# gmum/3d-point-clouds-autocomplete

Measured on AMD Instinct MI355X. Metric: train-step point-clouds/sec at B=64, N=2048 (Chamfer+EMD), higher is better.
Workload: dtype f32 storage / accumulation / results; matrix products formed from f16 x2 (bf16 x3) pieces of the fp32 operands — NOT IEEE-fp32 products: the all-fp32-kernel step is `value_strict_fp32`

## Files before the change

3d-point-clouds-autocomplete_amd/csrc/conv_pp.hip:

```cpp
#include "hp_common.h"
#include "hp_conv_split.h"
#include <algorithm>
#include <cstdlib>
#include <type_traits>

namespace {

typedef _Float16 f16x8 __attribute__((ext_vector_type(8)));
typedef _Float16 f16x4 __attribute__((ext_vector_type(4)));
typedef _Float16 f16x2 __attribute__((ext_vector_type(2)));
typedef float f32x16 __attribute__((ext_vector_type(16)));
typedef float f32x4 __attribute__((ext_vector_type(4)));
typedef unsigned int u32x4 __attribute__((ext_vector_type(4)));
typedef unsigned int u32x2 __attribute__((ext_vector_type(2)));

constexpr int kTarget = 14;
constexpr int kExpMax = HP_PP_EXP_MAX;

__device__ __forceinline__ int frexp_exp(unsigned bits) {
    const int E = (int)((bits >> 23) & 0xff);
    return E ? E - 126 : 0;
}
__device__ __forceinline__ float pow2f(int e) {
    e = max(-126, min(127, e));
// ... 286 lines not shown
                            }
                        }
                    const float ov = __shfl_xor(best, 32, 64);
                    const int oi = __shfl_xor(bi, 32, 64);
                    if (ov > best || (ov == best && oi < bi)) {
                        best = ov;
                        bi = oi;
                    }
                    if (h == 0) {
                        cmax[(long)tile128 * p.N + col] = best;
                        cidx[(long)tile128 * p.N + col] = bi % p.group_rows;
                    }
                }
            }
            continue;
        }

        float m = 0.f;
        const float usA = pow2f(-ex), floor_v = p.relu ? 0.f : -__builtin_inff();
#pragma unroll
        for (int j = 0; j < TN; ++j)
#pragma unroll
            for (int e = 0; e < 16; e += 4) {
                const int cl = wn * 32 * TN + j * 32 + kmap(e, h);
                const f32x4 us4 = *reinterpret_cast<const f32x4*>(tab + cl), bv4 = *reinterpret_cast<const f32x4*>(tab + BN + cl);
#pragma unroll
                for (int u = 0; u < 4; ++u) {
                    const float us = us4[u] * usA;
#pragma unroll
                    for (int i = 0; i < 4; ++i) {
                        const float v = fmaxf(__builtin_fmaf(acc[i][j][e + u], us, bv4[u]), floor_v);
                        acc[i][j][e + u] = v;
                        m = fmaxf(m, fabsf(v));
                    }
                }
            }
#pragma unroll
        for (int o = 1; o < 64; o <<= 1) m = fmaxf(m, __shfl_xor(m, o, 64));
        if (lane == 0) xch[wid] = m;
        __syncthreads();
        m = fmaxf(fmaxf(xch[wm * 4], xch[wm * 4 + 1]), fmaxf(xch[wm * 4 + 2], xch[wm * 4 + 3]));
        const int eo = block_exp(m);
        if (wn == 0 && lane == 0 && row0 + wm * 128 < M) p.cexp[z * p.sWs + (long)tile128 * p.tiles_n + tile_n] = eo;
        const float sx = pow2f(eo);
        unsigned char* Cb = reinterpret_cast<unsigned char*>(p.C) + z * p.sWs * 4;
        const long crow = (long)p.N * 4;
#pragma unroll
        for (int i = 0; i < 4; ++i) {
            const int row = row0 + wm * 128 + i * 32 + r;
#pragma unroll
            for (int j = 0; j < TN; ++j) {
                unsigned H[4][2], L[4][2];
#pragma unroll
                for (int q = 0; q < 4; ++q)
#pragma unroll
                    for (int pr = 0; pr < 2; ++pr) {
                        const float x0 = acc[i][j][4 * q + 2 * pr] * sx, x1 = acc[i][j][4 * q + 2 * pr + 1] * sx;
                        H[q][pr] = pack2((_Float16)x0, (_Float16)x1);
                        L[q][pr] = lo_pair(x0, x1, H[q][pr]);
                    }
                unsigned char* line = Cb + (long)row * crow + (long)((col0 + wn * 32 * TN) / 32 + j) * 128 + (h << 4);
#pragma unroll
                for (int q = 0; q < 4; q += 2) {
#pragma unroll
                    for (int pr = 0; pr < 2; ++pr) {
                        auto s1 = __builtin_amdgcn_permlane32_swap(H[q][pr], H[q + 1][pr], false, false);
                        H[q][pr] = s1[0];
                        H[q + 1][pr] = s1[1];
                        auto s2 = __builtin_amdgcn_permlane32_swap(L[q][pr], L[q + 1][pr], false, false);
                        L[q][pr] = s2[0];
                        L[q + 1][pr] = s2[1];
                    }
                    if (row < M) {
                        *reinterpret_cast<u32x4*>(line + q * 16) = u32x4{H[q][0], H[q][1], H[q + 1][0], H[q + 1][1]};
                        *reinterpret_cast<u32x4*>(line + 64 + q * 16) = u32x4{L[q][0], L[q][1], L[q + 1][0], L[q + 1][1]};
                    }
                }
            }
        }
        __syncthreads();
    }
}

__global__ __launch_bounds__(256) void conv1_pp_kernel(const float* __restrict__ x, long sXz, const float* __restrict__ W, long sWz,
                                                       const float* __restrict__ b, long sBz, _Float16* __restrict__ h, int* __restrict__ hexp,
                                                       long sWs, long R) {
    __shared__ float smax[4];
    const int z = blockIdx.y;
    x += z * sXz; W += z * sWz; b += z * sBz;
    unsigned char* hb = reinterpret_cast<unsigned char*>(h) + z * sWs * 4;
    hexp += z * sWs;
    const int c4 = (threadIdx.x & 15) * 4;
    float w0[4], w1[4], w2[4], bb[4];
#pragma unroll
    for (int u = 0; u < 4; ++u) {
        w0[u] = W[(c4 + u) * 3];
        w1[u] = W[(c4 + u) * 3 + 1];
        w2[u] = W[(c4 + u) * 3 + 2];
        bb[u] = b[c4 + u];
    }
    for (long tile = blockIdx.x; tile * 128 < R; tile += gridDim.x) {
        const long base = tile * 128 + (threadIdx.x >> 4);
        float xv[8][3];
#pragma unroll
        for (int q = 0; q < 8; ++q) {
            const long row = min(base + 16 * q, R - 1);
            xv[q][0] = x[row * 3];
            xv[q][1] = x[row * 3 + 1];
            xv[q][2] = x[row * 3 + 2];
        }
        float o[8][4];
        float m = 0.f;
#pragma unroll
        for (int q = 0; q < 8; ++q)
#pragma unroll
            for (int u = 0; u < 4; ++u) {
                const float v = __builtin_fmaf(xv[q][2], w2[u], __builtin_fmaf(xv[q][1], w1[u], __builtin_fmaf(xv[q][0], w0[u], 0.f)));
                o[q][u] = fmaxf(v + bb[u], 0.f);
                if (base + 16 * q < R) m = fmaxf(m, o[q][u]);
            }
        m = hp::wave_max(m);
        __syncthreads();
        if ((threadIdx.x & 63) == 0) smax[threadIdx.x >> 6] = m;
        __syncthreads();
        const int eo = block_exp(fmaxf(fmaxf(smax[0], smax[1]), fmaxf(smax[2], smax[3])));
        if (threadIdx.x == 0) hexp[tile] = eo;
        const float sx = pow2f(eo);
#pragma unroll
        for (int q = 0; q < 8; ++q) {
            const long row = base + 16 * q;
            f16x4 hi, lo;
#pragma unroll
            for (int u = 0; u < 4; ++u) {
                const float xs = o[q][u] * sx;
                const _Float16 hh = (_Float16)xs;
                hi[u] = hh;
                lo[u] = (_Float16)(xs - (float)hh);
            }
            if (row < R) {
                unsigned char* line = hb + row * 256 + (c4 >> 5) * 128 + (c4 & 31) * 2;
                *reinterpret_cast<f16x4*>(line) = hi;
                *reinterpret_cast<f16x4*>(line + 64) = lo;
            }
        }
    }
}

__global__ __launch_bounds__(256) void pp_pack_kernel(const float* __restrict__ X, long M, int C, int cb, _Float16* __restrict__ P,
                                                      int* __restrict__ pexp) {
    __shared__ float smax[4];
    const int ncb = C / cb, blk = blockIdx.x % ncb;
    const long tile = blockIdx.x / ncb, r0 = tile * 128;
    const int rows = (int)min((long)128, M - r0);
    const int per_row = cb / 4;
    float m = 0.f;
    for (int i = threadIdx.x; i < rows * per_row; i += 256) {
        const int rr = i / per_row, c = blk * cb + (i % per_row) * 4;
        const f32x4 v = *reinterpret_cast<const f32x4*>(X + (r0 + rr) * C + c);
        m = fmaxf(fmaxf(m, fmaxf(fabsf(v[0]), fabsf(v[1]))), fmaxf(fabsf(v[2]), fabsf(v[3])));
    }
    m = hp::wave_max(m);
    if ((threadIdx.x & 63) == 0) smax[threadIdx.x >> 6] = m;
    __syncthreads();
    const int eo = block_exp(fmaxf(fmaxf(smax[0], smax[1]), fmaxf(smax[2], smax[3])));
    if (threadIdx.x == 0) pexp[tile * ncb + blk] = eo;
    const float sx = pow2f(eo);
    unsigned char* Pb = reinterpret_cast<unsigned char*>(P);
    for (int i = threadIdx.x; i < rows * per_row; i += 256) {
        const int rr = i / per_row, c = blk * cb + (i % per_row) * 4;
        const f32x4 v = *reinterpret_cast<const f32x4*>(X + (r0 + rr) * C + c);
        f16x4 hi, lo;
#pragma unroll
        for (int u = 0; u < 4; ++u) {
            const float xs = v[u] * sx;
            const _Float16 hh = (_Float16)xs;
            hi[u] = hh;
            lo[u] = (_Float16)(xs - (float)hh);
        }
        unsigned char* line = Pb + (r0 + rr) * (long)C * 4 + (c >> 5) * 128 + (c & 31) * 2;
        *reinterpret_cast<f16x4*>(line) = hi;
        *reinterpret_cast<f16x4*>(line + 64) = lo;
    }
}

__global__ __launch_bounds__(256) void pp_unpack_kernel(const _Float16* P, const int* __restrict__ pexp, long M, int C, int cb,
                                                        float* out, const int* __restrict__ fmt) {
    if (fmt && *fmt != HP_PP_FMT_P) return;
    const long nlines = M * (C / 32);
    const int ncb = C / cb;
    for (long ln = (long)blockIdx.x * 256 + threadIdx.x; ln < nlines; ln += (long)gridDim.x * 256) {
        const long row = ln / (C / 32);
        const int kt = (int)(ln % (C / 32));
        const u32x4* src = reinterpret_cast<const u32x4*>(reinterpret_cast<const unsigned char*>(P) + ln * 128);
        u32x4 w[8];
#pragma unroll
        for (int q = 0; q < 8; ++q) w[q] = src[q];
        const float us = pow2f(-pexp[(row >> 7) * ncb + (kt * 32) / cb]);
        f32x4* dst = reinterpret_cast<f32x4*>(reinterpret_cast<unsigned char*>(out) + ln * 128);
#pragma unroll
        for (int q = 0; q < 4; ++q) {
            const f16x8 hi = __builtin_bit_cast(f16x8, w[q]), lo = __builtin_bit_cast(f16x8, w[q + 4]);
            f32x4 a, b;
#pragma unroll
            for (int u = 0; u < 4; ++u) {
                a[u] = ((float)hi[u] + (float)lo[u]) * us;
                b[u] = ((float)hi[u + 4] + (float)lo[u + 4]) * us;
            }
            dst[2 * q] = a;
            dst[2 * q + 1] = b;
        }
    }
}

__global__ void pp_set_fmt_kernel(int* fmt, int v) { *fmt = v; }

hp::Switch g_presplit("HP_CONV_PRESPLIT", 1);

int pp_bn(int N) { return N >= 256 ? 256 : 128; }
int launch_pp(int mode, int n, const PpParams& p, hipStream_t stream) {
    const int bn = pp_bn(p.N);
    if (p.N % bn || p.K % 64 || p.M <= 0) return -1;
    PpParams q = p;
    q.tiles_n = p.N / bn;
    constexpr int kCus = 256;
    const bool small = mode == 0 && bn == 128;
    const int bm = small ? 128 : 256;
    const long tiles = (long)((p.M + bm - 1) / bm) * q.tiles_n;
    const int per_cu = small ? 2 : 1;
    long wgs = std::min<long>(tiles, kCus * per_cu / n > 0 ? kCus * per_cu / n : 1);
    const int mult = 8 * q.tiles_n / (q.tiles_n % 8 == 0 ? 8 : (8 % q.tiles_n == 0 ? q.tiles_n : 1));
    if (wgs >= mult) wgs = wgs / mult * mult;
    else wgs = (tiles >= q.tiles_n) ? q.tiles_n : wgs;
    const dim3 grid((unsigned)wgs, n);
    if (mode == 1) {
        if (bn == 256) hipLaunchKernelGGL((conv_pp_kernel<1, 2, 2>), grid, dim3(512), 0, stream, q);
        else hipLaunchKernelGGL((conv_pp_kernel<1, 1, 2>), grid, dim3(512), 0, stream, q);
    } else {
        if (bn == 256) hipLaunchKernelGGL((conv_pp_kernel<0, 2, 2>), grid, dim3(512), 0, stream, q);
        else hipLaunchKernelGGL((conv_pp_kernel<0, 1, 1>), grid, dim3(256), 0, stream, q);
    }
    HP_RETURN_LAST_ERROR();
}

}

bool hp_conv_presplit_enabled() { return g_presplit.get() != 0; }
int hp_conv_pp_ncb(int l) {
    static const int kC[5] = {0, 64, 128, 256, 512};
    return l <= 1 ? 1 : kC[l] / pp_bn(kC[l]);
}
HP_API int hp_conv_presplit_set(int on) { return g_presplit.set(on); }

static inline long pexp_off(int l, long tp) { return hp_conv_pp_exp_offset(l, tp); }

long hp_conv_pp_fmt_offset(long R) { return hp_conv_pp_exp_offset(5, hp_conv_split_tiles_pad(R)); }

int hp_conv_pp_layer1(int n, const float* x, long sXz, const float* W, long sWz, const float* b, long sBz, float* h1, float* area0,
                      long sWs, long R, hipStream_t stream) {
    const long tp = hp_conv_split_tiles_pad(R), blocks = (R + 127) / 128;
    hipLaunchKernelGGL(conv1_pp_kernel, dim3((unsigned)(blocks < 2048 ? blocks : 2048), n), dim3(256), 0, stream, x, sXz, W, sWz, b, sBz,
                       reinterpret_cast<_Float16*>(h1), reinterpret_cast<int*>(area0 + pexp_off(1, tp)), sWs, R);
    HP_RETURN_LAST_ERROR();
}

int hp_conv_pp_layer(int l, int n, const float* X, const float* bias, long sBiasz, float* C, float* area0, long sWs, long M,
                     float* cmax, int* cidx, int group_rows, hipStream_t stream) {
    static const int kRowsL[5] = {0, 128, 384, 896, 1408};
    static const long kWOffL[4] = {0, 8192, 40960, 172032};
    static const int kKL[4] = {64, 128, 256, 512};
    if (l < 2 || l > 5 || M <= 0) return -1;
    const long tp = hp_conv_split_tiles_pad(M);
    PpParams p{};
    p.A = reinterpret_cast<const _Float16*>(X);
    p.aexp = reinterpret_cast<const int*>(area0 + pexp_off(l - 1, tp));
    p.K = kKL[l - 2];
    p.a_ncb = hp_conv_pp_ncb(l - 1);
    p.a_kb_steps = p.K / 32 / p.a_ncb;
    p.Whl = reinterpret_cast<const _Float16*>(area0 + HP_CS_HI_OFF) + 2 * kWOffL[l - 2];
    p.wexp = reinterpret_cast<const int*>(area0 + HP_CS_WEXP_OFF) + kRowsL[l - 2];
    p.bias = bias; p.sBiasz = sBiasz;
    p.C = reinterpret_cast<_Float16*>(C);
    p.cexp = l < 5 ? reinterpret_cast<int*>(area0 + pexp_off(l, tp)) : nullptr;
    p.cmax = cmax; p.cidx = cidx;
    p.sWs = sWs;
    p.M = (int)M; p.N = kRowsL[l - 1] - kRowsL[l - 2];
    p.relu = l < 5; p.group_rows = group_rows;
    return launch_pp(l == 5 ? 1 : 0, n, p, stream);
}

int hp_conv_pp_mark(int n, float* area0, long sWs, long R, int fmt, hipStream_t stream) {
    for (int z = 0; z < n; ++z)
        hipLaunchKernelGGL(pp_set_fmt_kernel, dim3(1), dim3(1), 0, stream, reinterpret_cast<int*>(area0 + z * sWs + hp_conv_pp_fmt_offset(R)), fmt);
    HP_RETURN_LAST_ERROR();
}

int hp_conv_pp_unpack_ws(float* ws, long R, hipStream_t stream) {
    static const int kC[4] = {64, 128, 256, 512};
    const long tp = hp_conv_split_tiles_pad(R);
    float* area = ws + R * (64 + 128 + 256 + 512 + 512);
    int* fmt = reinterpret_cast<int*>(area + hp_conv_pp_fmt_offset(R));
    float* hl = ws;
    for (int l = 1; l <= 4; ++l) {
        const int C = kC[l - 1];
        const long lines = R * (C / 32);
        const unsigned blocks = (unsigned)std::min<long>((lines + 255) / 256, 8192);
        hipLaunchKernelGGL(pp_unpack_kernel, dim3(blocks), dim3(256), 0, stream, reinterpret_cast<const _Float16*>(hl),
                           reinterpret_cast<const int*>(area + pexp_off(l, tp)), R, C, C / hp_conv_pp_ncb(l), hl, fmt);
        hl += R * C;
    }
    hipLaunchKernelGGL(pp_set_fmt_kernel, dim3(1), dim3(1), 0, stream, fmt, HP_PP_FMT_F32);
    HP_RETURN_LAST_ERROR();
}

HP_API long hp_gemm_pp_workspace_floats(long M, int N, int K) {
    const long tiles = (M + 127) / 128;
    return M * K + tiles * 16 + N + (long)N * K + M * N + tiles * 16 + 2 * tiles * N + 64;
}
namespace {
struct PpWs {
    float *xp, *xexp, *wexp, *wp, *cp, *cexp, *cmax, *cidx;
};
PpWs pp_ws(float* ws, long M, int N, int K) {
    const long tiles = (M + 127) / 128;
    PpWs w;
    w.xp = ws;
    w.xexp = w.xp + M * K;
    w.wexp = w.xexp + tiles * 16;
    w.wp = w.wexp + N;
    w.cp = w.wp + (long)N * K;
    w.cexp = w.cp + M * N;
    w.cmax = w.cexp + tiles * 16;
    w.cidx = w.cmax + tiles * N;
    return w;
}
}
int hp_split_rows_launch(const float* W, int N, int K, float* hl, float* wexp, hipStream_t stream);

HP_API int hp_gemm_pp_prepare(long M, int N, int K, int xcb, const float* X, const float* W, float* ws, hipStream_t stream) {
    HP_CHECK_ARG(M > 0 && N > 0 && K > 0 && N % 128 == 0 && K % 32 == 0 && K <= 512 && xcb > 0 && K % xcb == 0 && xcb % 32 == 0 &&
                 K / xcb <= 16 && X && W && ws);
    const PpWs w = pp_ws(ws, M, N, K);
    const long tiles = (M + 127) / 128;
    hipLaunchKernelGGL(pp_pack_kernel, dim3((unsigned)(tiles * (K / xcb))), dim3(256), 0, stream, X, M, K, xcb,
                       reinterpret_cast<_Float16*>(w.xp), reinterpret_cast<int*>(w.xexp));
// ... 42 lines not shown
```

3d-point-clouds-autocomplete_amd/csrc/hp_conv_split.h:

```cpp
#pragma once
#include <hip/hip_runtime.h>

#define HP_CS_WEXP_OFF 0L
#define HP_CS_HI_OFF 1408L
#define HP_CS_LO_OFF (HP_CS_HI_OFF + 434176L / 2)
#define HP_CS_AMAX_OFF (HP_CS_LO_OFF + 434176L / 2)

#define HP_PP_EXP_MAX 54
#define HP_PP_FMT_F32 0
#define HP_PP_FMT_P 0x50464d54

inline long hp_conv_split_tiles_pad(long R) { return ((R + 127) / 128 + 3) / 4 * 4; }
long hp_conv_split_area_floats(long R);
bool hp_conv_split_enabled();
int hp_conv_split_prep(int n, const float* const* W0, const float* const* W1, float* area0, long sArea, long R, int fmt, hipStream_t stream);
int hp_conv_split_layer1(int n, const float* x, long sXz, const float* W, long sWz, const float* b, long sBz, float* h1, long sHz,
                         float* area0, long sArea, long R, hipStream_t stream);
int hp_conv_split_layer(int l, int n, const float* X, long sXz, const float* bias, long sBiasz, float* C, long sCz, float* area0,
                        long sArea, long M, int relu, int colmax, float* cmax, int* cidx, int group_rows, hipStream_t stream);

bool hp_conv_presplit_enabled();
long hp_conv_pp_fmt_offset(long R);
int hp_conv_pp_layer1(int n, const float* x, long sXz, const float* W, long sWz, const float* b, long sBz, float* h1, float* area0,
                      long sWs, long R, hipStream_t stream);
int hp_conv_pp_layer(int l, int n, const float* X, const float* bias, long sBiasz, float* C, float* area0, long sWs, long M,
                     float* cmax, int* cidx, int group_rows, hipStream_t stream);
int hp_conv_pp_mark(int n, float* area0, long sWs, long R, int fmt, hipStream_t stream);
int hp_conv_pp_unpack_ws(float* ws, long R, hipStream_t stream);
inline long hp_conv_pp_exp_offset(int l, long tp) { return HP_CS_AMAX_OFF + 4 * tp + (long)(l - 1) * 4 * tp; }
int hp_conv_pp_ncb(int l);
```

3d-point-clouds-autocomplete_amd/csrc/model.hip:

```cpp
#include "hp_common.h"
#include "hp_gemm.h"
#include "hp_conv_split.h"
#include "hp_model.h"
#include "hp_skinny.h"
#include "hp_enc_bwd.h"
#include <algorithm>
#include <cstdlib>

extern "C" int hp_gemm_f32(const HpGemmDesc* d, hipStream_t stream);
extern "C" int hp_gemm_tile_rows(const HpGemmDesc* d);
extern "C" int hp_colsum_f32(int batch, int M, int N, const float* X, long sXz, int ldx, const float* mask, long sMaskz,
                             int ldmask, float* out, long sOz, float* ws, hipStream_t stream);

namespace {

constexpr int kEnc[6] = {3, 64, 128, 256, 512, 512};
constexpr int kTrunk[5] = {64, 128, 512, 1024, 2048};
constexpr long kSplitWs = 4L << 20;

#define TRY(x)            \
    do {                  \
        int _rc = (x);    \
        if (_rc) return _rc; \
    } while (0)
// ... 425 lines not shown
};
int enc_tail_backward_skinny(int B, int out_size, int n, const EncTailBwd* t, hipStream_t stream) {
    if (B > 64 || out_size % 32) return -2;
    HpSkProgram pr{};
    const int S2 = sk_ranges(512, 512 / 32, 4);
    if (S2 == 1) return -2;
    int S[2], nh[2];
    for (int e = 0; e < n; ++e) {
        nh[e] = t[e].dlv ? 2 : 1;
        S[e] = sk_ranges(out_size, 512 / 32, 4 / nh[e]);
        if (nh[e] * S[e] == 1) return -2;
    }
    for (int e = 0; e < n; ++e) {
        for (int hd = 0; hd < nh[e]; ++hd) {
            HpSkOp& op = pr.op[pr.nops++];
            op.type = HP_SK_X; op.phase = 0;
            op.a.p = hd ? t[e].dlv : t[e].dmu; op.a.S = 1; op.a.ld = hd ? out_size : t[e].dmu_ld;
            op.w = hd ? t[e].w->std_w : t[e].w->mu_w; op.w_ld = 512;
            op.M = B; op.N = out_size; op.K = 512; op.CL = out_size / S[e];
            op.out = t[e].slabs + (long)hd * S[e] * 64 * 512; op.out_slab = 64L * 512; op.out_ld = 512;
        }
        for (int hd = 0; hd < nh[e]; ++hd) {
            HpSkOp& op = pr.op[pr.nops++];
            op.type = HP_SK_W; op.phase = 0;
            op.a.p = hd ? t[e].dlv : t[e].dmu; op.a.S = 1; op.a.ld = hd ? out_size : t[e].dmu_ld;
            op.w = t[e].f; op.w_ld = 512;
            op.out = hd ? t[e].gr->std_w : t[e].gr->mu_w; op.out_ld = 512; op.rsum = hd ? t[e].gr->std_b : t[e].gr->mu_b;
            op.M = B; op.N = out_size; op.K = 512;
        }
    }
    for (int e = 0; e < n; ++e) {
        float* s2 = t[e].slabs + (long)nh[e] * S[e] * 64 * 512;
        HpSkOp& xf = pr.op[pr.nops++];
        xf.type = HP_SK_X; xf.phase = 1;
        xf.a.p = t[e].slabs; xf.a.slab = 64L * 512; xf.a.S = nh[e] * S[e]; xf.a.ld = 512; xf.a.mask = t[e].f; xf.a.ldm = 512;
        xf.a.mat = t[e].dfc; xf.a.ldmat = 512;
        xf.w = t[e].w->fc_w; xf.w_ld = 512;
        xf.M = B; xf.N = 512; xf.K = 512; xf.CL = 512 / S2;
        xf.out = s2; xf.out_slab = 64L * 512; xf.out_ld = 512;
    }
    for (int e = 0; e < n; ++e) {
        float* s2 = t[e].slabs + (long)nh[e] * S[e] * 64 * 512;
        HpSkOp& fin = pr.op[pr.nops++];
        fin.type = HP_SK_FIN; fin.phase = 2;
        fin.a.p = s2; fin.a.slab = 64L * 512; fin.a.S = S2; fin.a.ld = 512;
        fin.out = t[e].dg; fin.out_ld = 512;
        fin.M = B; fin.N = 512; fin.K = 1;
        HpSkOp& wf = pr.op[pr.nops++];
        wf.type = HP_SK_W; wf.phase = 2;
        wf.a.p = t[e].dfc; wf.a.S = 1; wf.a.ld = 512;
        wf.w = t[e].g; wf.w_ld = 512;
        wf.out = t[e].gr->fc_w; wf.out_ld = 512; wf.rsum = t[e].gr->fc_b;
        wf.M = B; wf.N = 512; wf.K = 512;
    }
    return hp_skinny_run(&pr, stream);
}
}

HP_API long hp_encoder_forward_workspace_floats(int B, int Np) { return enc_fwd_ws(B, Np); }
HP_API long hp_encoder_backward_workspace_floats(int B, int out_size) { return enc_bwd_ws(B, out_size); }

namespace {
int encoder_forward_impl(int B, int Np, int out_size, int n, const HpEncoderIO* io, hipStream_t stream) {
    const long R = (long)B * Np;
    Op op{stream, nullptr};
    const HpEncoderIO& e0 = io[0];
    const HpEncoderIO& e1 = io[n - 1];
    auto dz = [&](const float* a0, const float* a1) { return n > 1 ? (long)(a1 - a0) : 0L; };
    float* h[6];
    h[0] = nullptr;
    h[1] = e0.ws;
    for (int l = 2; l <= 5; ++l) h[l] = h[l - 1] + R * kEnc[l - 1];
    const long sWs = dz(e0.ws, e1.ws);
    const bool split = hp_conv_split_enabled();
    float* area = h[5] + R * 512;
    const bool presplit = split && hp_conv_presplit_enabled() && Np % 128 == 0;
    if (split) {
        const float* W0[4] = {e0.w->conv_w[1], e0.w->conv_w[2], e0.w->conv_w[3], e0.w->conv_w[4]};
        const float* W1[4] = {e1.w->conv_w[1], e1.w->conv_w[2], e1.w->conv_w[3], e1.w->conv_w[4]};
        TRY(hp_conv_split_prep(n, W0, W1, area, sWs, R, presplit ? HP_PP_FMT_P : HP_PP_FMT_F32, stream));
    } else {
        TRY(hp_conv_pp_mark(n, area, sWs, R, HP_PP_FMT_F32, stream));
    }
    if (presplit) {
        TRY(hp_conv_pp_layer1(n, e0.x, dz(e0.x, e1.x), e0.w->conv_w[0], dz(e0.w->conv_w[0], e1.w->conv_w[0]), e0.w->conv_b[0],
                              dz(e0.w->conv_b[0], e1.w->conv_b[0]), h[1], area, sWs, R, stream));
        for (int l = 2; l <= 4; ++l)
            TRY(hp_conv_pp_layer(l, n, h[l - 1], e0.w->conv_b[l - 1], dz(e0.w->conv_b[l - 1], e1.w->conv_b[l - 1]), h[l], area, sWs, R,
                                 nullptr, nullptr, 0, stream));
    } else if (split) {
        TRY(hp_conv_split_layer1(n, e0.x, dz(e0.x, e1.x), e0.w->conv_w[0], dz(e0.w->conv_w[0], e1.w->conv_w[0]), e0.w->conv_b[0],
                                 dz(e0.w->conv_b[0], e1.w->conv_b[0]), h[1], sWs, area, sWs, R, stream));
        for (int l = 2; l <= 4; ++l)
            TRY(hp_conv_split_layer(l, n, h[l - 1], sWs, e0.w->conv_b[l - 1], dz(e0.w->conv_b[l - 1], e1.w->conv_b[l - 1]), h[l], sWs,
                                    area, sWs, R, 1, 0, nullptr, nullptr, 0, stream));
    } else {
        const float* in = e0.x;
        long sIn = dz(e0.x, e1.x);
        for (int l = 1; l <= 4; ++l) {
            TRY(op.lin_fwd(in, sIn, kEnc[l - 1], e0.w->conv_w[l - 1], dz(e0.w->conv_w[l - 1], e1.w->conv_w[l - 1]),
                           e0.w->conv_b[l - 1], dz(e0.w->conv_b[l - 1], e1.w->conv_b[l - 1]), h[l], sWs, kEnc[l], (int)R, kEnc[l],
                           kEnc[l - 1], n, true));
            in = h[l];
            sIn = sWs;
        }
    }
    HpGemmDesc d5{};
    d5.A = h[4]; d5.sAz = sWs; d5.sAi = 512; d5.sAk = 1;
    d5.B = e0.w->conv_w[4]; d5.sBz = dz(e0.w->conv_w[4], e1.w->conv_w[4]); d5.sBk = 1; d5.sBj = 512;
    d5.bias = e0.w->conv_b[4]; d5.sBiasz = dz(e0.w->conv_b[4], e1.w->conv_b[4]);
    d5.sCz = sWs;
    d5.M = (int)R; d5.N = 512; d5.K = 512; d5.batch = n;
    d5.flags = HP_GEMM_BIAS | HP_GEMM_COLMAX;
    d5.group_rows = Np;
    const int tr = split ? 128 : hp_gemm_tile_rows(&d5);
    long tail_off = -1;
    if (tr > 0 && Np % tr == 0) {
        const long tiles = R / tr;
        d5.cmax = h[5];
        d5.cidx = reinterpret_cast<int*>(h[5] + tiles * 512);
        if (R * 512 - up4(2 * tiles * 512) >= 4L * 64 * 512 + 8L * 64 * out_size) tail_off = up4(2 * tiles * 512);
        if (presplit)
            TRY(hp_conv_pp_layer(5, n, h[4], d5.bias, d5.sBiasz, nullptr, area, sWs, R, d5.cmax, d5.cidx, Np, stream));
        else if (split)
            TRY(hp_conv_split_layer(5, n, h[4], sWs, d5.bias, d5.sBiasz, nullptr, sWs, area, sWs, R, 0, 1, d5.cmax, d5.cidx, Np, stream));
        else
            TRY(hp_gemm_f32(&d5, stream));
        hipLaunchKernelGGL(colmax_tiles_kernel, dim3(2, B, n), dim3(256), 0, stream, d5.cmax, d5.cidx, Np / tr, tr, 512, io[0].g,
                           io[0].argidx, sWs, io[n - 1].g, io[n - 1].argidx);
    } else {
        if (split)
            TRY(hp_conv_split_layer(5, n, h[4], sWs, d5.bias, d5.sBiasz, h[5], sWs, area, sWs, R, 0, 0, nullptr, nullptr, 0, stream));
        else
            TRY(op.lin_fwd(h[4], sWs, 512, e0.w->conv_w[4], d5.sBz, e0.w->conv_b[4], d5.sBiasz, h[5], sWs, 512, (int)R, 512, 512, n,
                           false));
        for (int z = 0; z < n; ++z)
            hipLaunchKernelGGL(colmax_kernel, dim3(512 / 64, B), dim3(256), 0, stream, h[5] + z * sWs, Np, 512, io[z].g,
                               io[z].argidx);
    }
    int sk = -2;
    if (hp_skinny_enabled() && tail_off >= 0 && B <= 64) {
        EncTail t[2];
        for (int z = 0; z < n; ++z) t[z] = EncTail{io[z].g, io[z].w, io[z].is_vae, io[z].f, io[z].mu, io[z].lv, h[5] + z * sWs + tail_off,
                           (!io[z].is_vae && io[z].out_ld > 0) ? io[z].out_ld : out_size};
        sk = enc_tail_forward_skinny(B, out_size, n, t, stream);
    }
    if (sk != -2) TRY(sk);
    for (int z = 0; z < n; ++z) {
        const HpEncoderIO& e = io[z];
        if (sk == -2) {
            TRY(op.lin_fwd(e.g, 0, 512, e.w->fc_w, 0, e.w->fc_b, 0, e.f, 0, 512, B, 512, 512, 1, true));
            TRY(op.lin_fwd(e.f, 0, 512, e.w->mu_w, 0, e.w->mu_b, 0, e.mu, 0, (!e.is_vae && e.out_ld > 0) ? e.out_ld : out_size, B,
                           out_size, 512, 1, false));
            if (e.is_vae)
                TRY(op.lin_fwd(e.f, 0, 512, e.w->std_w, 0, e.w->std_b, 0, e.lv, 0, out_size, B, out_size, 512, 1, false));
        }
        if (e.is_vae) {
            const long nel = (long)B * out_size;
            hipLaunchKernelGGL(vae_head_fwd_kernel, dim3((int)cdiv(nel, 256)), dim3(256), 0, stream, nel, e.eps, e.mu, e.lv, e.z,
                               out_size, e.out_ld > 0 ? e.out_ld : out_size, e.explv);
        }
    }
    HP_RETURN_LAST_ERROR();
}

bool encoder_io_ok(const HpEncoderIO& e) {
    return e.x && e.w && e.argidx && e.g && e.f && e.mu && e.ws &&
// ... 651 lines not shown
```

include/hyperpocket_hip.h:

```cpp
#ifndef HYPERPOCKET_HIP_H
#define HYPERPOCKET_HIP_H

#ifdef __cplusplus
extern "C" {
#endif

typedef struct ihipStream_t* hpStream_t;


int hp_nndistance(int b, int n, const float* xyz, int m, const float* xyz2, float* result, int* result_i,
                  float* result2, int* result2_i, hpStream_t stream);

int hp_nndistancegrad(int b, int n, const float* xyz1, int m, const float* xyz2, const float* grad_dist1,
                      const int* idx1, const float* grad_dist2, const int* idx2, float* grad_xyz1, float* grad_xyz2,
                      hpStream_t stream);

int hp_approxmatch(int b, int n, int m, const float* xyz1, const float* xyz2, float* match, float* temp,
                   hpStream_t stream);
long hp_approxmatch_workspace_floats(int b, int n, int m);
int hp_approxmatch_ws(int b, int n, int m, const float* xyz1, const float* xyz2, float* match, float* temp, float* ws,
                      hpStream_t stream);
int hp_emd_set_rows_per_lane(int rows1, int rows2, int grad2);
int hp_emd_set_final_derive(int on);
int hp_emd_set_chains(int chains);
// ... 44 lines not shown
    const float* bias;
    const float* mask;
    const float* add;
    float* ws;
    long sAz, sBz, sCz, sBiasz, sMaskz, sAddz;
    long sAi, sAk, sBk, sBj;
    int ldc, ldmask, ldadd;
    int M, N, K, batch;
    int ksplit;
    int flags;
    float* cmax;
    int* cidx;
    int group_rows;
    float* rsum;
    long sRsumz;
    const int* dyn_count;
    int dyn_kind;
} HpGemmDesc;

long hp_gemm_workspace_floats(const HpGemmDesc* d);
int hp_gemm_tile_rows(const HpGemmDesc* d);
int hp_gemm_f32(const HpGemmDesc* d , hpStream_t stream);
long hp_colsum_workspace_floats(int batch, int M, int N);
int hp_colsum_f32(int batch, int M, int N, const float* X, long sXz, int ldx, const float* mask, long sMaskz,
                  int ldmask, float* out, long sOz, float* ws , hpStream_t stream);

#define HP_MAX_HEADS 8
#define HP_MAX_TN_LAYERS 8

typedef struct HpEncoderWeights {
    const float* conv_w[5];
    const float* conv_b[5];
    const float* fc_w;
    const float* fc_b;
    const float* mu_w;
    const float* mu_b;
    const float* std_w;
    const float* std_b;
} HpEncoderWeights;

typedef struct HpEncoderGrads {
    float* conv_w[5];
    float* conv_b[5];
    float* fc_w;
    float* fc_b;
    float* mu_w;
    float* mu_b;
    float* std_w;
    float* std_b;
} HpEncoderGrads;

typedef struct HpHyperWeights {
    const float* trunk_w[5];
    const float* trunk_b[5];
    int n_heads;
    int head_out[HP_MAX_HEADS];
    const float* head_w[HP_MAX_HEADS];
    const float* head_b[HP_MAX_HEADS];
} HpHyperWeights;

typedef struct HpHyperGrads {
    float* trunk_w[5];
    float* trunk_b[5];
    float* head_w[HP_MAX_HEADS];
    float* head_b[HP_MAX_HEADS];
} HpHyperGrads;

long hp_encoder_forward_workspace_floats(int B, int Np);
int hp_encoder_forward(int B, int Np, const float* x, const HpEncoderWeights* w, int out_size, int is_vae,
                       const float* eps, int* argidx, float* g, float* f, float* mu, float* lv, float* z, float* explv,
                       float* ws, hpStream_t stream);
typedef struct HpEncoderIO {
    const float* x;
    const HpEncoderWeights* w;
    const float* eps;
    int* argidx;
    float *g, *f, *mu, *lv, *z, *explv, *ws;
    int is_vae;
    int out_ld;
} HpEncoderIO;
int hp_encoder_forward_pair(int B, int Np, int out_size, const HpEncoderIO* io , hpStream_t stream);
int hp_encoder_workspace_to_f32(int B, int Np, float* ws, hpStream_t stream);
int hp_conv_presplit_set(int on);
long hp_gemm_pp_workspace_floats(long M, int N, int K);
int hp_gemm_pp_prepare(long M, int N, int K, int xcb, const float* X, const float* W, float* ws, hpStream_t stream);
int hp_gemm_pp_run(long M, int N, int K, int xcb, const float* bias, int relu, int mode, int group_rows, float* ws, hpStream_t stream);
int hp_gemm_pp_unpack(long M, int N, int K, const float* ws, float* C, hpStream_t stream);
int hp_gemm_pp_partials(long M, int N, int K, const float* ws, float* cmax, int* cidx, hpStream_t stream);
long hp_encoder_backward_workspace_floats(int B, int out_size);
int hp_encoder_backward(int B, int Np, const float* x, const HpEncoderWeights* w, int out_size, int is_vae,
                        const float* eps, const int* argidx, const float* g, const float* f, const float* lv,
                        const float* grad_out, const float* grad_mu, const float* grad_explv, const HpEncoderGrads* grads,
                        float* ws, const float* fwd_ws, int dedup, hpStream_t stream);
int hp_encoder_backward_ld(int B, int Np, const float* x, const HpEncoderWeights* w, int out_size, int is_vae,
                           const float* eps, const int* argidx, const float* g, const float* f, const float* lv,
                           const float* grad_out, int grad_out_ld, const float* grad_mu, const float* grad_explv,
                           const HpEncoderGrads* grads, float* ws, const float* fwd_ws, int dedup, hpStream_t stream);
typedef struct HpEncoderBwdIO {
    const float* x;
    const HpEncoderWeights* w;
    const float* eps;
    const int* argidx;
    const float *g, *f, *lv;
    const float *grad_out, *grad_mu, *grad_explv;
    const HpEncoderGrads* gr;
    float* ws;
    const float* fwd_ws;
    int is_vae;
    int grad_out_ld;
} HpEncoderBwdIO;
int hp_encoder_backward_pair(int B, int Np, int out_size, const HpEncoderBwdIO* io , int dedup, hpStream_t stream);
int hp_encoder_backward_pair_ordered(int B, int Np, int out_size, const HpEncoderBwdIO* io , int dedup, hpStream_t stream,
                                     hpStream_t after);
int hp_encoder_backward_set_fused(int on);
int hp_encoder_backward_set_chain_f16(int on);
int hp_conv_split_set(int on);
long hp_gemm_f16x2_workspace_floats(long M, int N, int K);
int hp_gemm_f16x2_prepare(long M, int N, int K, const float* X, const float* W, float* ws, hpStream_t stream);
int hp_gemm_f16x2_run(long M, int N, int K, const float* X, const float* bias, float* C, int relu, const float* ws, hpStream_t stream);

int hp_hypernet_set_heads_stream(int on);
long hp_hypernet_saved_floats(int B);
int hp_hypernet_forward(int B, int in_size, const float* latent, const HpHyperWeights* w, float* t, float* theta,
                        int theta_ld, hpStream_t stream);
long hp_hypernet_backward_workspace_floats(int B);
int hp_hypernet_backward(int B, int in_size, const float* latent, const HpHyperWeights* w, const float* t,
                         const float* grad_theta, int theta_ld, const HpHyperGrads* grads, float* grad_latent ,
                         float* ws, hpStream_t stream);
int hp_hypernet_backward_ordered(int B, int in_size, const float* latent, const HpHyperWeights* w, const float* t,
                                 const float* grad_theta, int theta_ld, const HpHyperGrads* grads, float* grad_latent ,
                                 float* ws, hpStream_t stream, hpStream_t after);
long hp_hypernet_t5_offset(int B);
long hp_hypernet_heads_dw_workspace_floats(void);
int hp_hypernet_heads_dw_rows(int Kc, int rows, int r0, const float* dtheta_all, int theta_ld, const float* t5_all,
                              float* dW_rows, float* ws, hpStream_t stream);

int hp_hypernet_heads_dw_adam(int Kc, int rows, int r0, const float* dtheta_all, int theta_ld, const float* t5_all,
                              float* W_rows, float* m_rows, float* v_rows, float lr, float beta1, float beta2, float eps,
                              int step, hpStream_t stream);
int hp_hypernet_heads_dw_adam_bg(int Kc, int rows, int r0, const float* dtheta_all, int theta_ld, const float* t5_all,
                                 float* W_rows, float* m_rows, float* v_rows, float lr, float beta1, float beta2, float eps,
                                 int step, int cus, hpStream_t stream);

int hp_skinny_set_enabled(int on);

long hp_target_theta_size(int n_hidden, const int* channels);
long hp_target_saved_floats(int B, int N, int n_hidden, const int* channels);
int hp_target_forward(int B, int N, int n_hidden, const int* channels, const float* theta, int theta_ld, const float* pts,
                      float* acts, float* y, hpStream_t stream);
long hp_target_backward_workspace_floats(int B, int N, int n_hidden, const int* channels);
int hp_target_backward(int B, int N, int n_hidden, const int* channels, const float* theta, int theta_ld, const float* pts,
                       const float* acts, const float* grad_y, float* grad_theta, float* ws, hpStream_t stream);

int hp_target_fused_supported(int n_hidden, const int* channels);
long hp_target_fused_workspace_floats(int B, int N);
int hp_target_fused_set_f16(int on);
int hp_target_fused_forward(int B, int N, const float* theta, int theta_ld, const float* pts, float* y, hpStream_t stream);
int hp_target_fused_backward(int B, int N, const float* theta, int theta_ld, const float* pts, const float* grad_y,
                             float* grad_theta, float* ws, hpStream_t stream);

int hp_sample_points(long total, float coef, unsigned long long seed, unsigned long long offset, float* out,
                     hpStream_t stream);
int hp_slice_clouds(int B, int N, int target, const float* pts, unsigned long long seed, int max_rounds, float* part_a,
                    float* part_b, float* plane, int* status, hpStream_t stream);
int hp_slice_clouds_planes(int B, int N, int target, const float* pts, const double* planes, int R, float* part_a,
                           float* part_b, int* plane_idx, int* status, hpStream_t stream);
// ... 14 lines not shown
```

Baseline: 24110.

## Fuse encoder conv layers 1-3 into one kernel with LDS-resident activations

Adds a single kernel that computes conv layer 1 (3->64), then layers 2 (64->128) and 3 (128->256) with f16 split MFMA for a 128-row tile, keeping intermediate split activations in shared memory instead of reloading them from global memory between launches. It still writes h1/h2/h3 and per-tile exponents to global memory for the backward pass. The goal is to remove two kernel launches and the global reads of h1/h2. In exchange the kernel uses about 64KB of LDS and 512 threads with a waves-per-eu hint, which may limit occupancy, and it uses one block per tile with no persistent scheduling.

```diff
diff --git a/3d-point-clouds-autocomplete_amd/csrc/conv_pp.hip b/3d-point-clouds-autocomplete_amd/csrc/conv_pp.hip
--- a/3d-point-clouds-autocomplete_amd/csrc/conv_pp.hip
+++ b/3d-point-clouds-autocomplete_amd/csrc/conv_pp.hip
@@ -392,6 +392,11 @@
     }
 }
 
+__device__ __forceinline__ float conv1_value(float x0, float x1, float x2, float w0, float w1, float w2, float b) {
+    const float v = __builtin_fmaf(x2, w2, __builtin_fmaf(x1, w1, __builtin_fmaf(x0, w0, 0.f)));
+    return fmaxf(v + b, 0.f);
+}
+
 __global__ __launch_bounds__(256) void conv1_pp_kernel(const float* __restrict__ x, long sXz, const float* __restrict__ W, long sWz,
                                                        const float* __restrict__ b, long sBz, _Float16* __restrict__ h, int* __restrict__ hexp,
                                                        long sWs, long R) {
@@ -425,8 +430,7 @@
         for (int q = 0; q < 8; ++q)
 #pragma unroll
             for (int u = 0; u < 4; ++u) {
-                const float v = __builtin_fmaf(xv[q][2], w2[u], __builtin_fmaf(xv[q][1], w1[u], __builtin_fmaf(xv[q][0], w0[u], 0.f)));
-                o[q][u] = fmaxf(v + bb[u], 0.f);
+                o[q][u] = conv1_value(xv[q][0], xv[q][1], xv[q][2], w0[u], w1[u], w2[u], bb[u]);
                 if (base + 16 * q < R) m = fmaxf(m, o[q][u]);
             }
         m = hp::wave_max(m);
@@ -451,6 +455,265 @@
                 unsigned char* line = hb + row * 256 + (c4 >> 5) * 128 + (c4 & 31) * 2;
                 *reinterpret_cast<f16x4*>(line) = hi;
                 *reinterpret_cast<f16x4*>(line + 64) = lo;
+            }
+        }
+    }
+}
+
+struct Fuse13Params {
+    const float* x;  long sXz;
+    const float* W1; long sW1z;
+    const float* b1; long sB1z;
+    const float* b2; long sB2z;
+    const float* b3; long sB3z;
+    unsigned char *h1, *h2, *h3;
+    int *e1, *e2, *e3;
+    const unsigned char *W2p, *W3p;
+    const int *wexp2, *wexp3;
+    long sWs, R;
+};
+
+__device__ __forceinline__ void mode0_bias_relu(f32x16& a, const float* tab, int nch, int cl, int h, float usA, float& m) {
+#pragma unroll
+    for (int e = 0; e < 16; e += 4) {
+        const int c = cl + kmap(e, h);
+        const f32x4 us4 = *reinterpret_cast<const f32x4*>(tab + c), bv4 = *reinterpret_cast<const f32x4*>(tab + nch + c);
+#pragma unroll
+        for (int u = 0; u < 4; ++u) {
+            const float v = fmaxf(__builtin_fmaf(a[e + u], us4[u] * usA, bv4[u]), 0.f);
+            a[e + u] = v;
+            m = fmaxf(m, fabsf(v));
+        }
+    }
+}
+__device__ __forceinline__ void split_chunks(const f32x16& a, float sx, u32x4& hi0, u32x4& hi2, u32x4& lo0, u32x4& lo2) {
+    unsigned H[4][2], L[4][2];
+#pragma unroll
+    for (int q = 0; q < 4; ++q)
+#pragma unroll
+        for (int pr = 0; pr < 2; ++pr) {
+            const float x0 = a[4 * q + 2 * pr] * sx, x1 = a[4 * q + 2 * pr + 1] * sx;
+            H[q][pr] = pack2((_Float16)x0, (_Float16)x1);
+            L[q][pr] = lo_pair(x0, x1, H[q][pr]);
+        }
+#pragma unroll
+    for (int q = 0; q < 4; q += 2)
+#pragma unroll
+        for (int pr = 0; pr < 2; ++pr) {
+            auto s1 = __builtin_amdgcn_permlane32_swap(H[q][pr], H[q + 1][pr], false, false);
+            H[q][pr] = s1[0];
+            H[q + 1][pr] = s1[1];
+            auto s2 = __builtin_amdgcn_permlane32_swap(L[q][pr], L[q + 1][pr], false, false);
+            L[q][pr] = s2[0];
+            L[q + 1][pr] = s2[1];
+        }
+    hi0 = u32x4{H[0][0], H[0][1], H[1][0], H[1][1]};
+    hi2 = u32x4{H[2][0], H[2][1], H[3][0], H[3][1]};
+    lo0 = u32x4{L[0][0], L[0][1], L[1][0], L[1][1]};
+    lo2 = u32x4{L[2][0], L[2][1], L[3][0], L[3][1]};
+}
+__device__ __forceinline__ float block_max8(float m, float* slot, int lane, int wid) {
+#pragma unroll
+    for (int o = 1; o < 64; o <<= 1) m = fmaxf(m, __shfl_xor(m, o, 64));
+    if (lane == 0) slot[wid] = m;
+    __syncthreads();
+    m = slot[0];
+#pragma unroll
+    for (int w = 1; w < 8; ++w) m = fmaxf(m, slot[w]);
+    return m;
+}
+
+__global__ __launch_bounds__(512) __attribute__((amdgpu_waves_per_eu(4))) void conv13_pp_kernel(const Fuse13Params p) {
+    constexpr int kImgKt = 128 * 128;
+    __shared__ __attribute__((aligned(1024))) unsigned char img[4 * kImgKt];
+    __shared__ __attribute__((aligned(16))) float tab2[2 * 128], tab3[2 * 256];
+    __shared__ float xch[3][8];
+    const int z = blockIdx.y, tile = blockIdx.x;
+    const long R = p.R, row0 = (long)tile * 128, zs = z * p.sWs;
+    const int tid = threadIdx.x, lane = tid & 63, wid = tid >> 6, r = lane & 31, h = lane >> 5, swz = (r >> 1) & 7;
+    auto slot = [](int c, int s) { return ((c ^ s) << 4); };
+
+    const int c2 = (wid & 3) * 32, rh = wid >> 2;
+    f16x8 b2[2][2][2];
+    {
+        const unsigned char* w = p.W2p + zs * 4 + (long)(c2 + r) * 256;
+#pragma unroll
+        for (int kt = 0; kt < 2; ++kt)
+#pragma unroll
+            for (int t = 0; t < 2; ++t) {
+                b2[kt][t][0] = *reinterpret_cast<const f16x8*>(w + kt * 128 + (2 * t + h) * 16);
+                b2[kt][t][1] = *reinterpret_cast<const f16x8*>(w + kt * 128 + (4 + 2 * t + h) * 16);
+            }
+    }
+    if (tid < 128) {
+        tab2[tid] = pow2f(-p.wexp2[zs + tid]);
+        tab2[128 + tid] = p.b2[z * p.sB2z + tid];
+    }
+    if (tid < 256) {
+        tab3[tid] = pow2f(-p.wexp3[zs + tid]);
+        tab3[256 + tid] = p.b3[z * p.sB3z + tid];
+    }
+
+    int e1;
+    {
+        const int c4 = (tid & 15) * 4, rg = tid >> 4;
+        const float* x = p.x + z * p.sXz;
+        const float* W = p.W1 + z * p.sW1z;
+        const float* b = p.b1 + z * p.sB1z;
+        float w0[4], w1[4], w2[4], bb[4], xv[4][3];
+#pragma unroll
+        for (int u = 0; u < 4; ++u) {
+            w0[u] = W[(c4 + u) * 3];
+            w1[u] = W[(c4 + u) * 3 + 1];
+            w2[u] = W[(c4 + u) * 3 + 2];
+            bb[u] = b[c4 + u];
+        }
+#pragma unroll
+        for (int q = 0; q < 4; ++q) {
+            const long row = min(row0 + rg + 32 * q, R - 1);
+            xv[q][0] = x[row * 3];
+            xv[q][1] = x[row * 3 + 1];
+            xv[q][2] = x[row * 3 + 2];
+        }
+        float o[4][4], m = 0.f;
+#pragma unroll
+        for (int q = 0; q < 4; ++q)
+#pragma unroll
+            for (int u = 0; u < 4; ++u) {
+                o[q][u] = conv1_value(xv[q][0], xv[q][1], xv[q][2], w0[u], w1[u], w2[u], bb[u]);
+                if (row0 + rg + 32 * q < R) m = fmaxf(m, o[q][u]);
+            }
+        e1 = block_exp(block_max8(m, xch[0], lane, wid));
+        if (tid == 0) p.e1[zs + tile] = e1;
+        const float sx = pow2f(e1);
+        unsigned char* hb = p.h1 + zs * 4;
+        const int ck = (c4 & 31) >> 3;
+#pragma unroll
+        for (int q = 0; q < 4; ++q) {
+            const int rl = rg + 32 * q;
+            f16x4 hi, lo;
+#pragma unroll
+            for (int u = 0; u < 4; ++u) {
+                const float xs = o[q][u] * sx;
+                const _Float16 hh = (_Float16)xs;
+                hi[u] = hh;
+                lo[u] = (_Float16)(xs - (float)hh);
+            }
+            if (row0 + rl < R) {
+                unsigned char* line = hb + (row0 + rl) * 256 + (c4 >> 5) * 128 + (c4 & 31) * 2;
+                *reinterpret_cast<f16x4*>(line) = hi;
+                *reinterpret_cast<f16x4*>(line + 64) = lo;
+            }
+            unsigned char* li = img + (c4 >> 5) * kImgKt + rl * 128 + (c4 & 7) * 2;
+            const int s = (rl >> 1) & 7;
+            *reinterpret_cast<f16x4*>(li + slot(ck, s)) = hi;
+            *reinterpret_cast<f16x4*>(li + slot(ck + 4, s)) = lo;
+        }
+        __syncthreads();
+    }
+
+    int e2;
+    {
+        f32x16 acc[2];
+#pragma unroll
+        for (int i = 0; i < 2; ++i)
+#pragma unroll
+            for (int e = 0; e < 16; ++e) acc[i][e] = 0.f;
+#pragma unroll
+        for (int kt = 0; kt < 2; ++kt)
+#pragma unroll
+            for (int t = 0; t < 2; ++t) {
+                f16x8 ah[2], al[2];
+#pragma unroll
+                for (int i = 0; i < 2; ++i) {
+                    const unsigned char* a = img + kt * kImgKt + (rh * 64 + i * 32 + r) * 128;
+                    ah[i] = *reinterpret_cast<const f16x8*>(a + slot(2 * t + h, swz));
+                    al[i] = *reinterpret_cast<const f16x8*>(a + slot(4 + 2 * t + h, swz));
+                }
+#pragma unroll
+                for (int pr = 0; pr < 3; ++pr)
+#pragma unroll
+                    for (int i = 0; i < 2; ++i)
+                        acc[i] = __builtin_amdgcn_mfma_f32_32x32x16_f16(pr == 1 ? b2[kt][t][1] : b2[kt][t][0], pr == 2 ? al[i] : ah[i],
+                                                                       acc[i], 0, 0, 0);
+            }
+        float m = 0.f;
+        const float usA = pow2f(-e1);
+#pragma unroll
+        for (int i = 0; i < 2; ++i) mode0_bias_relu(acc[i], tab2, 128, c2, h, usA, m);
+        e2 = block_exp(block_max8(m, xch[1], lane, wid));
+        if (tid == 0) p.e2[zs + tile] = e2;
+        const float sx = pow2f(e2);
+#pragma unroll
+        for (int i = 0; i < 2; ++i) {
+            const int rl = rh * 64 + i * 32 + r;
+            u32x4 H0, H2, L0, L2;
+            split_chunks(acc[i], sx, H0, H2, L0, L2);
+            if (row0 + rl < R) {
+                unsigned char* line = p.h2 + zs * 4 + (row0 + rl) * 512 + (c2 >> 5) * 128 + (h << 4);
+                *reinterpret_cast<u32x4*>(line) = H0;
+                *reinterpret_cast<u32x4*>(line + 32) = H2;
+                *reinterpret_cast<u32x4*>(line + 64) = L0;
+                *reinterpret_cast<u32x4*>(line + 96) = L2;
+            }
+            unsigned char* li = img + (c2 >> 5) * kImgKt + rl * 128;
+            *reinterpret_cast<u32x4*>(li + slot(h, swz)) = H0;
+            *reinterpret_cast<u32x4*>(li + slot(2 + h, swz)) = H2;
+            *reinterpret_cast<u32x4*>(li + slot(4 + h, swz)) = L0;
+            *reinterpret_cast<u32x4*>(li + slot(6 + h, swz)) = L2;
+        }
+        __syncthreads();
+    }
+
+    {
+        const int c3 = wid * 32;
+        const unsigned char* w = p.W3p + zs * 4 + (long)(c3 + r) * 512;
+        f32x16 acc[4];
+#pragma unroll
+        for (int i = 0; i < 4; ++i)
+#pragma unroll
+            for (int e = 0; e < 16; ++e) acc[i][e] = 0.f;
+#pragma unroll
+        for (int kt = 0; kt < 4; ++kt)
+#pragma unroll
+            for (int t = 0; t < 2; ++t) {
+                const f16x8 bh = *reinterpret_cast<const f16x8*>(w + kt * 128 + (2 * t + h) * 16);
+                const f16x8 bl = *reinterpret_cast<const f16x8*>(w + kt * 128 + (4 + 2 * t + h) * 16);
+#pragma unroll
+                for (int ip = 0; ip < 2; ++ip) {
+                    f16x8 ah[2], al[2];
+#pragma unroll
+                    for (int u = 0; u < 2; ++u) {
+                        const unsigned char* a = img + kt * kImgKt + ((2 * ip + u) * 32 + r) * 128;
+                        ah[u] = *reinterpret_cast<const f16x8*>(a + slot(2 * t + h, swz));
+                        al[u] = *reinterpret_cast<const f16x8*>(a + slot(4 + 2 * t + h, swz));
+                    }
+#pragma unroll
+                    for (int pr = 0; pr < 3; ++pr)
+#pragma unroll
+                        for (int u = 0; u < 2; ++u)
+                            acc[2 * ip + u] = __builtin_amdgcn_mfma_f32_32x32x16_f16(pr == 1 ? bl : bh, pr == 2 ? al[u] : ah[u],
+                                                                                     acc[2 * ip + u], 0, 0, 0);
+                }
+            }
+        float m = 0.f;
+        const float usA = pow2f(-e2);
+#pragma unroll
+        for (int i = 0; i < 4; ++i) mode0_bias_relu(acc[i], tab3, 256, c3, h, usA, m);
+        const int e3 = block_exp(block_max8(m, xch[2], lane, wid));
+        if (tid == 0) p.e3[zs + tile] = e3;
+        const float sx = pow2f(e3);
+#pragma unroll
+        for (int i = 0; i < 4; ++i) {
+            const long row = row0 + i * 32 + r;
+            u32x4 H0, H2, L0, L2;
+            split_chunks(acc[i], sx, H0, H2, L0, L2);
+            if (row < R) {
+                unsigned char* line = p.h3 + zs * 4 + row * 1024 + (c3 >> 5) * 128 + (h << 4);
+                *reinterpret_cast<u32x4*>(line) = H0;
+                *reinterpret_cast<u32x4*>(line + 32) = H2;
+                *reinterpret_cast<u32x4*>(line + 64) = L0;
+                *reinterpret_cast<u32x4*>(line + 96) = L2;
             }
         }
     }
@@ -525,6 +788,7 @@
 __global__ void pp_set_fmt_kernel(int* fmt, int v) { *fmt = v; }
 
 hp::Switch g_presplit("HP_CONV_PRESPLIT", 1);
+hp::Switch g_fuse13("HP_CONV_FUSE13", 1);
 
 int pp_bn(int N) { return N >= 256 ? 256 : 128; }
 int launch_pp(int mode, int n, const PpParams& p, hipStream_t stream) {
@@ -560,6 +824,8 @@
     return l <= 1 ? 1 : kC[l] / pp_bn(kC[l]);
 }
 HP_API int hp_conv_presplit_set(int on) { return g_presplit.set(on); }
+bool hp_conv_fuse13_enabled() { return g_fuse13.get() != 0; }
+HP_API int hp_conv_fuse13_set(int on) { return g_fuse13.set(on); }
 
 static inline long pexp_off(int l, long tp) { return hp_conv_pp_exp_offset(l, tp); }
 
@@ -570,6 +836,32 @@
     const long tp = hp_conv_split_tiles_pad(R), blocks = (R + 127) / 128;
     hipLaunchKernelGGL(conv1_pp_kernel, dim3((unsigned)(blocks < 2048 ? blocks : 2048), n), dim3(256), 0, stream, x, sXz, W, sWz, b, sBz,
                        reinterpret_cast<_Float16*>(h1), reinterpret_cast<int*>(area0 + pexp_off(1, tp)), sWs, R);
+    HP_RETURN_LAST_ERROR();
+}
+
+int hp_conv_pp_layers13(int n, const float* x, long sXz, const float* W1, long sW1z, const float* b1, long sB1z, const float* b2,
+                        long sB2z, const float* b3, long sB3z, float* h1, float* area0, long sWs, long R, hipStream_t stream) {
+    const long tp = hp_conv_split_tiles_pad(R), tiles = (R + 127) / 128;
+    if (R <= 0 || tiles > 0x7fffffffL) return -1;
+    Fuse13Params p{};
+    p.x = x; p.sXz = sXz;
+    p.W1 = W1; p.sW1z = sW1z;
+    p.b1 = b1; p.sB1z = sB1z;
+    p.b2 = b2; p.sB2z = sB2z;
+    p.b3 = b3; p.sB3z = sB3z;
+    p.h1 = reinterpret_cast<unsigned char*>(h1);
+    p.h2 = reinterpret_cast<unsigned char*>(h1 + R * 64);
+    p.h3 = reinterpret_cast<unsigned char*>(h1 + R * (64 + 128));
+    p.e1 = reinterpret_cast<int*>(area0 + pexp_off(1, tp));
+    p.e2 = reinterpret_cast<int*>(area0 + pexp_off(2, tp));
+    p.e3 = reinterpret_cast<int*>(area0 + pexp_off(3, tp));
+    const unsigned char* pieces = reinterpret_cast<const unsigned char*>(area0 + HP_CS_HI_OFF);
+    p.W2p = pieces;
+    p.W3p = pieces + 128 * 64 * 4;
+    p.wexp2 = reinterpret_cast<const int*>(area0 + HP_CS_WEXP_OFF);
+    p.wexp3 = p.wexp2 + 128;
+    p.sWs = sWs; p.R = R;
+    hipLaunchKernelGGL(conv13_pp_kernel, dim3((unsigned)tiles, n), dim3(512), 0, stream, p);
     HP_RETURN_LAST_ERROR();
 }
 
diff --git a/3d-point-clouds-autocomplete_amd/csrc/hp_conv_split.h b/3d-point-clouds-autocomplete_amd/csrc/hp_conv_split.h
--- a/3d-point-clouds-autocomplete_amd/csrc/hp_conv_split.h
+++ b/3d-point-clouds-autocomplete_amd/csrc/hp_conv_split.h
@@ -23,6 +23,9 @@
 long hp_conv_pp_fmt_offset(long R);
 int hp_conv_pp_layer1(int n, const float* x, long sXz, const float* W, long sWz, const float* b, long sBz, float* h1, float* area0,
                       long sWs, long R, hipStream_t stream);
+bool hp_conv_fuse13_enabled();
+int hp_conv_pp_layers13(int n, const float* x, long sXz, const float* W1, long sW1z, const float* b1, long sB1z, const float* b2,
+                        long sB2z, const float* b3, long sB3z, float* h1, float* area0, long sWs, long R, hipStream_t stream);
 int hp_conv_pp_layer(int l, int n, const float* X, const float* bias, long sBiasz, float* C, float* area0, long sWs, long M,
                      float* cmax, int* cidx, int group_rows, hipStream_t stream);
 int hp_conv_pp_mark(int n, float* area0, long sWs, long R, int fmt, hipStream_t stream);
diff --git a/3d-point-clouds-autocomplete_amd/csrc/model.hip b/3d-point-clouds-autocomplete_amd/csrc/model.hip
--- a/3d-point-clouds-autocomplete_amd/csrc/model.hip
+++ b/3d-point-clouds-autocomplete_amd/csrc/model.hip
@@ -531,7 +531,14 @@
     } else {
         TRY(hp_conv_pp_mark(n, area, sWs, R, HP_PP_FMT_F32, stream));
     }
-    if (presplit) {
+    const bool fuse13 = presplit && hp_conv_fuse13_enabled();
+    if (fuse13) {
+        TRY(hp_conv_pp_layers13(n, e0.x, dz(e0.x, e1.x), e0.w->conv_w[0], dz(e0.w->conv_w[0], e1.w->conv_w[0]), e0.w->conv_b[0],
+                                dz(e0.w->conv_b[0], e1.w->conv_b[0]), e0.w->conv_b[1], dz(e0.w->conv_b[1], e1.w->conv_b[1]),
+                                e0.w->conv_b[2], dz(e0.w->conv_b[2], e1.w->conv_b[2]), h[1], area, sWs, R, stream));
+        TRY(hp_conv_pp_layer(4, n, h[3], e0.w->conv_b[3], dz(e0.w->conv_b[3], e1.w->conv_b[3]), h[4], area, sWs, R, nullptr, nullptr, 0,
+                             stream));
+    } else if (presplit) {
         TRY(hp_conv_pp_layer1(n, e0.x, dz(e0.x, e1.x), e0.w->conv_w[0], dz(e0.w->conv_w[0], e1.w->conv_w[0]), e0.w->conv_b[0],
                               dz(e0.w->conv_b[0], e1.w->conv_b[0]), h[1], area, sWs, R, stream));
         for (int l = 2; l <= 4; ++l)
diff --git a/include/hyperpocket_hip.h b/include/hyperpocket_hip.h
--- a/include/hyperpocket_hip.h
+++ b/include/hyperpocket_hip.h
@@ -150,6 +150,7 @@
 int hp_encoder_forward_pair(int B, int Np, int out_size, const HpEncoderIO* io , hpStream_t stream);
 int hp_encoder_workspace_to_f32(int B, int Np, float* ws, hpStream_t stream);
 int hp_conv_presplit_set(int on);
+int hp_conv_fuse13_set(int on);
 long hp_gemm_pp_workspace_floats(long M, int N, int K);
 int hp_gemm_pp_prepare(long M, int N, int K, int xcb, const float* X, const float* W, float* ws, hpStream_t stream);
 int hp_gemm_pp_run(long M, int N, int K, int xcb, const float* bias, int relu, int mode, int group_rows, float* ws, hpStream_t stream);
```

New measurement: 24270 (median of 6 runs). Within noise of the previous version (+0.6%).
